# deezer/musicFPaugment

Measured on AMD Instinct MI355X. Metric: 8s/8kHz clips/sec (STFT+UNet+peak-pick), higher is better.
Workload: dtype bf16x3 (fp32 operands split into bf16 hi+lo, fp32 accumulate); 1 GPU; STFT(512/256,f64) -> UNet(1,1) eval forward (bf16x3 MFMA, formula weights) -> Audfprint peak-pick; 8 s / 8 kHz clips, 257x251 spectrograms; parallelism=clip-sharded x1, no data-path collective

## Files before the change

musicfpaugment_amd/csrc/mfpa_conv_tile.h:

```cpp
#pragma once
#include <hip/hip_runtime.h>

#include <type_traits>
#include <utility>

namespace mfpa_tile {

typedef float floatx16 __attribute__((ext_vector_type(16)));
typedef float floatx4 __attribute__((ext_vector_type(4)));
typedef float f32x4 __attribute__((ext_vector_type(4)));
typedef float f32x2 __attribute__((ext_vector_type(2)));
typedef __bf16 bf16x8 __attribute__((ext_vector_type(8)));
typedef __bf16 bf16x4 __attribute__((ext_vector_type(4)));
typedef __bf16 bf16x2 __attribute__((ext_vector_type(2)));

constexpr int KC = 32;

template <int CTRL>
__device__ __forceinline__ float dpp_row_add(float v) {
  return v + __int_as_float(__builtin_amdgcn_update_dpp(0, __float_as_int(v), CTRL, 0xf, 0xf, false));
}

template <int SLOTS, int LEFT, int I = 0>
__device__ __forceinline__ void pin_reads() {
  if constexpr (I < SLOTS && LEFT > 0) {
    constexpr int k = (LEFT + (SLOTS - I) - 1) / (SLOTS - I);
    __builtin_amdgcn_sched_group_barrier(0x008, 1, 0);
    __builtin_amdgcn_sched_group_barrier(0x100, k, 0);
    pin_reads<SLOTS, LEFT - k, I + 1>();
  }
}
constexpr int pin_read_slots(int slots, int left) {
  int used = 0;
  for (int i = 0; i < slots && left > 0; ++i) {
    left -= (left + (slots - i) - 1) / (slots - i);
    ++used;
  }
  return used;
}

__device__ __forceinline__ void split_bf16x3(f32x2 x, unsigned& hi, unsigned& lo) {
  hi = __builtin_bit_cast(unsigned, __builtin_convertvector(x, bf16x2));
  const f32x2 r = {x[0] - __uint_as_float(hi << 16), x[1] - __uint_as_float(hi & 0xffff0000u)};
  lo = __builtin_bit_cast(unsigned, __builtin_convertvector(r, bf16x2));
}

__device__ __forceinline__ void mfma_bf16x3(floatx16& acc, bf16x8 ah, bf16x8 al, bf16x8 bh, bf16x8 bl) {
  acc = __builtin_amdgcn_mfma_f32_32x32x16_bf16(al, bh, acc, 0, 0, 0);
  acc = __builtin_amdgcn_mfma_f32_32x32x16_bf16(ah, bl, acc, 0, 0, 0);
  acc = __builtin_amdgcn_mfma_f32_32x32x16_bf16(ah, bh, acc, 0, 0, 0);
}

template <int FIRST, class F, int... I, class... A>
__device__ __forceinline__ void each_index_impl(F&& f, std::integer_sequence<int, I...>, A&&... a) {
  (f(std::integral_constant<int, FIRST + I>{}, a...), ...);
}
template <int N, int FIRST = 0, class F, class... A>
__device__ __forceinline__ void each_index(F&& f, A&&... a) {
  each_index_impl<FIRST>(f, std::make_integer_sequence<int, N>{}, a...);
}

namespace role_split {
constexpr int PH = 8, PW = 32, HPW = PW + 2, HPH = PH + 2, HP = HPW * HPH;
constexpr int THREADS = 512, LTHREADS = 256;
constexpr int SPP = KC / 4;
constexpr int PPI = LTHREADS / SPP;
constexpr int A_F4 = (HP + PPI - 1) / PPI;
constexpr int HPS = A_F4 * PPI;
constexpr int PLANE = ((HPS * 16 + 255) / 256) * 256;
constexpr int HLS = 4 * PLANE + 256;
constexpr int STAGE = 2 * HLS;
constexpr int PT = 8;
constexpr int OUTBUF = PH * PW * 64 * 4;

__device__ __forceinline__ constexpr int plane_off(int hl, int kg) { return hl * HLS + kg * PLANE + (kg >> 1) * 128; }
}

}
```

musicfpaugment_amd/csrc/unet_up.hip:

```cpp
#include "mfpa_common.h"
#include "mfpa_conv_tile.h"
#include "mfpa_unet_args.h"

namespace mfpa_unet {
namespace {

using namespace mfpa_tile;
using namespace mfpa_tile::role_split;

constexpr int HALF = HPW / 2;
constexpr int LPH = PH / 2 + 2, LPW = PW / 2 + 2, LP = LPH * LPW;
constexpr int L_F4 = (LP + PPI - 1) / PPI;
constexpr int EPI_FLOATS = 64 + 16 * 64;

__device__ __forceinline__ int tile_of(int b, int i, int G, int ngrp) {
  if (ngrp == 1 && (G & 7) == 0) return i * G + (b & 7) * (G >> 3) + (b >> 3);
  return i * G + b;
}

__device__ __forceinline__ int bias_class(int v, int n2) { return v == 0 ? 0 : (v < n2 - 1 ? 1 : (v == n2 - 1 ? 2 : 3)); }

template <int PREC>
__global__ __launch_bounds__(THREADS, 1) void conv_up_kernel(UpArgs a) {
  extern __shared__ __attribute__((aligned(16))) char smem[];
// ... 129 lines not shown
        if (S.interior) each_index<A_F4>([&](auto IT) __attribute__((always_inline)) { issue_slot(S, ain, off0[decltype(IT)::value], std::true_type{}, SET, IT); });
        else each_index<A_F4>([&](auto IT) __attribute__((always_inline)) { issue_slot(S, ain, off0[decltype(IT)::value], std::false_type{}, SET, IT); });
      } else {
        if (S.interior) each_index<L_F4>([&](auto IT) __attribute__((always_inline)) { issue_slot(S, ain, off1[decltype(IT)::value], std::true_type{}, SET, IT); });
        else each_index<L_F4>([&](auto IT) __attribute__((always_inline)) { issue_slot(S, ain, off1[decltype(IT)::value], std::false_type{}, SET, IT); });
      }
    };
    auto split_all = [&](auto SET, int stage_off, bool from0) __attribute__((always_inline)) {
      each_index<L_F4>([&](auto IT) __attribute__((always_inline)) { split_slot(SET, IT, stage_off); });
      if (from0) each_index<A_F4 - L_F4, L_F4>([&](auto IT) __attribute__((always_inline)) { split_slot(SET, IT, stage_off); });
    };
    int qi = 0, qc = 0;
    Tile TQ = make_tile(tile_of(wgx, 0, G, ngrp));
    auto issue_next = [&](auto SET) __attribute__((always_inline)) {
      const Src S = make_src(TQ, qc);
      issue_all(S, TQ.ain, SET);
      if (++qc == nchunks) {
        qc = 0; ++qi;
        if (qi < owned) TQ = make_tile(tile_of(wgx, qi, G, ngrp));
      }
    };
    using SET0 = std::integral_constant<int, 0>;
    using SET1 = std::integral_constant<int, 1>;
    issue_next(SET0{});
    int par = 0;
    const int total = owned * nchunks;
    auto iteration = [&](int k, auto ISSUE_SET, auto SPLIT_SET) __attribute__((always_inline)) {
      if (k + 2 < total) issue_next(ISSUE_SET);
      __builtin_amdgcn_sched_barrier(0);
      if (k + 1 < total) split_all(SPLIT_SET, par * STAGE, ((k + 1) % nchunks) < nsk);
      if (k >= nchunks + 1 && (k - 1) % nchunks == 0) duty(tile_of(wgx, (k - 1) / nchunks - 1, G, ngrp));
      __syncthreads();
      par ^= 1;
    };
    for (int k = -1; k < total; k += 2) {
      iteration(k, SET1{}, SET0{});
      if (k + 1 < total) iteration(k + 1, SET0{}, SET1{});
    }
    __syncthreads();
    duty(tile_of(wgx, owned - 1, G, ngrp));
    return;
  }

  const int wm = wave & 1, wn = wave >> 1;
  const int p = lane & 15, g = lane >> 4;

  typedef typename std::conditional<PREC == 1, bf16x8, f32x4>::type frag_t;
  frag_t wq[4][2][2];
  const unsigned wrow = (unsigned)(a.Cout / 16), wcol = (unsigned)(n0 / 16 + 2 * wn);
  const __amdgpu_buffer_rsrc_t rs_skip = __builtin_amdgcn_make_buffer_rsrc(const_cast<float*>(a.w_skip), 0, (int)(9u * (unsigned)a.Cout * (unsigned)a.Cs * 4u), 0x00020000);
  const __amdgpu_buffer_rsrc_t rs_up = __builtin_amdgcn_make_buffer_rsrc(const_cast<float*>(a.w_up), 0, (int)(16u * (unsigned)a.Cout * (unsigned)a.Cl * 4u), 0x00020000);
  const int wlane = lane * 16;
  auto load_w_at = [&](__amdgpu_buffer_rsrc_t rs, unsigned blk, auto SLOT) __attribute__((always_inline)) {
    constexpr int slot = decltype(SLOT)::value;
    const int so = (int)__builtin_amdgcn_readfirstlane((int)(blk << 11));
    wq[slot][0][0] = __builtin_bit_cast(frag_t, __builtin_amdgcn_raw_buffer_load_b128(rs, wlane, so, 0));
    wq[slot][0][1] = __builtin_bit_cast(frag_t, __builtin_amdgcn_raw_buffer_load_b128(rs, wlane + 1024, so, 0));
    wq[slot][1][0] = __builtin_bit_cast(frag_t, __builtin_amdgcn_raw_buffer_load_b128(rs, wlane + 2048, so, 0));
    wq[slot][1][1] = __builtin_bit_cast(frag_t, __builtin_amdgcn_raw_buffer_load_b128(rs, wlane + 3072, so, 0));
  };
  auto load_w_skip = [&](int chunk, int tap, auto SLOT) __attribute__((always_inline)) {
    load_w_at(rs_skip, ((unsigned)tap * (unsigned)nsk + (unsigned)chunk) * wrow + wcol, SLOT);
  };
  auto load_w_up = [&](int chunk, int pair, int px, auto SLOT) __attribute__((always_inline)) {
    const unsigned t16 = (unsigned)((wm * 2 + px) * 4 + pair);
    load_w_at(rs_up, (t16 * (unsigned)nup + (unsigned)chunk) * wrow + wcol, SLOT);
  };
  struct XFrags { frag_t h[4], l[4]; };
  XFrags fx[2];
  const int pl0 = PREC == 1 ? plane_off(0, g) : plane_off(g >> 1, 2 * (g & 1));
  constexpr int SECOND = PREC == 1 ? HLS : PLANE;
  const int xb_skip = (wm * HPW + p) * 16 + pl0;
  const int xb_up = (wm * LPW + p) * 16 + pl0;
  constexpr int R_ALL = 0, R_FIRST = 1, R_SECOND = 2;
  auto read_at = [&](XFrags& f, const char* base, auto STRIDE, auto PART) __attribute__((always_inline)) {
    constexpr int stride = decltype(STRIDE)::value, part = decltype(PART)::value;
#pragma unroll
    for (int j = (part == R_SECOND ? 2 : 0); j < (part == R_FIRST ? 2 : 4); ++j) {
      const char* r = base + j * stride;
      f.l[j] = *reinterpret_cast<const frag_t*>(r + SECOND);
      f.h[j] = *reinterpret_cast<const frag_t*>(r);
    }
  };
  auto read_skip = [&](XFrags& f, const char* stage, auto TA, auto S, auto PART) __attribute__((always_inline)) {
    constexpr int ta = decltype(TA)::value, s = decltype(S)::value;
    read_at(f, stage + xb_skip + (ta * HPW + (s & 1) * HALF + (s >> 1)) * 16, std::integral_constant<int, 2 * HPW * 16>{}, PART);
  };
  auto read_up = [&](XFrags& f, const char* stage, auto TY, auto C, auto PART) __attribute__((always_inline)) {
    read_at(f, stage + xb_up + (decltype(TY)::value * LPW + decltype(C)::value) * 16, std::integral_constant<int, LPW * 16>{}, PART);
  };
  floatx4 acc[2][PT];
#pragma unroll
  for (int ct = 0; ct < 2; ++ct)
#pragma unroll
    for (int pt = 0; pt < PT; ++pt) acc[ct][pt] = floatx4{0.f, 0.f, 0.f, 0.f};
  floatx4 initv[2];
  auto mfma_half = [&](const XFrags& f, const frag_t (&w)[2][2], auto HALFI, auto FIRST) __attribute__((always_inline)) {
    constexpr int half = decltype(HALFI)::value;
    if constexpr (PREC == 0) {
#pragma unroll
      for (int s8 = 0; s8 < 8; ++s8)
#pragma unroll
        for (int ct = 0; ct < 2; ++ct)
#pragma unroll
          for (int i = 0; i < 4; ++i) {
            const float wv = (s8 < 4 ? w[ct][0] : w[ct][1])[s8 & 3], xv = (s8 < 4 ? f.h[i] : f.l[i])[s8 & 3];
            acc[ct][4 * half + i] = __builtin_amdgcn_mfma_f32_16x16x4f32(wv, xv, (decltype(FIRST)::value && s8 == 0) ? initv[ct] : acc[ct][4 * half + i], 0, 0, 0);
          }
      return;
    } else {
#pragma unroll
    for (int ct = 0; ct < 2; ++ct)
// ... 258 lines not shown
```

musicfpaugment_amd/csrc/unet_wd16.hip:

```cpp
#include "mfpa_common.h"
#include "mfpa_conv_tile.h"
#include "mfpa_unet_args.h"

namespace {

using namespace mfpa_tile;
using mfpa_unet::ConvArgs;

constexpr int wd16_bn(int wmw) { return 32 * (8 / wmw); }
constexpr bool wd16_persist(bool rows, int wmw, bool side, bool plain) { return wmw == 4 || (!rows && !side) || plain; }
template <int PH, int PW, bool IN16>
struct Wd16Lds {
  static constexpr int THREADS = 512;
  static constexpr int SPP = IN16 ? KC / 8 : KC / 4;
  static constexpr int HPW = PW + 2, HPH = PH + 2, HP = HPW * HPH;
  static constexpr int A_F4 = (HP * SPP + THREADS - 1) / THREADS;
  static constexpr int HPS = A_F4 * (THREADS / SPP);
  static constexpr int PLANE = ((HPS * 16 + 255) / 256) * 256;
  static constexpr int HLS = 4 * PLANE + 256;
  static constexpr int STAGE = 2 * HLS;
  static constexpr int TBL = 2 * A_F4 * THREADS;
  static constexpr int TBL_BYTES = 2 * ((HP * (KC / 4) + THREADS - 1) / THREADS) * THREADS * (int)sizeof(unsigned);
  static constexpr int RED = 2 * 256;
  static constexpr int epi_floats(int wmw) { return 2 * wd16_bn(wmw) + 64; }
  static constexpr int fixed_bytes(int wmw) { return 2 * STAGE + TBL_BYTES + epi_floats(wmw) * (int)sizeof(float); }
  __host__ __device__ static constexpr int plane_off(int hl, int kg) { return hl * HLS + kg * PLANE + (kg >> 1) * 128; }
  static_assert(TBL * (int)sizeof(unsigned) <= TBL_BYTES, "the kernel's table fits the launcher's");
};
static_assert(Wd16Lds<8, 32, false>::fixed_bytes(2) == 125184 && Wd16Lds<16, 16, false>::fixed_bytes(2) == 125184 &&
              Wd16Lds<8, 32, true>::fixed_bytes(2) == 125184 && Wd16Lds<16, 16, true>::fixed_bytes(2) == 125184, "LDS of the 128-channel tiles");
static_assert(Wd16Lds<8, 32, false>::fixed_bytes(4) == 124672 && Wd16Lds<8, 32, true>::fixed_bytes(4) == 124672, "LDS of the 64-channel tiles");


template <int PH, int PW, bool ROWS, int WMW = 2, bool SIDE = false, bool PLAIN = false, bool IN16 = false, bool AFF16 = false>
__global__ __launch_bounds__(512, 1) void conv_wd16_kernel(ConvArgs a) {
  static_assert(!IN16 || PLAIN, "a bf16 source feeds the plain-bf16 products");
  using G = Wd16Lds<PH, PW, IN16>;
  constexpr int SPP = G::SPP, HPW = G::HPW, HP = G::HP, A_F4 = G::A_F4, HLS = G::HLS, STAGE = G::STAGE, TBL = G::TBL;
  constexpr int ESZ = IN16 ? 2 : 4;
  constexpr int THREADS = G::THREADS, BN = wd16_bn(WMW), WPXW = 256 / WMW, TAPS = 9;
  static_assert((WMW == 2 || WMW == 4) && (!ROWS || WMW == 2), "wave grid");
  constexpr int BM = PH * PW;
  static_assert(BM == 256 && (PW == 32 || PW == 16), "two waves of 128 pixels: eight 16-pixel tiles each");
  constexpr int PT = WPXW / 16;
  static_assert(A_F4 <= TAPS - 3, "one halo staging slot per tap, taps 2 .. 7");

  extern __shared__ __attribute__((aligned(16))) char smem[];
  const int tid = threadIdx.x, lane = tid & 63, wave = tid >> 6;
  const int wm = wave % WMW, wn = __builtin_amdgcn_readfirstlane(wave / WMW);
  const int p = lane & 15, g = lane >> 4;

  constexpr bool PERSIST = wd16_persist(ROWS, WMW, SIDE, PLAIN);
  const int n0 = blockIdx.y * BN;
  const int Cin = a.C0 + a.C1;
  const int nchunks = Cin / KC;
  const int ntiles = a.tiles_x * a.tiles_y * a.B;

  const int aq = tid % SPP;
  unsigned* const aoffs0 = reinterpret_cast<unsigned*>(smem + 2 * STAGE);
#pragma unroll
  for (int it = 0; it < A_F4; ++it) {
    const int pix = tid / SPP + it * (THREADS / SPP);
    const int py = pix / HPW - 1, px = pix % HPW - 1;
    aoffs0[it * THREADS + tid] = (unsigned)((py * a.W + px) * a.C0 + (KC / SPP) * aq) * (unsigned)ESZ;
    aoffs0[(A_F4 + it) * THREADS + tid] = (unsigned)(((py - a.oy1) * a.W1 + (px - a.ox1)) * a.C1 + (KC / SPP) * aq) * (unsigned)ESZ;
  }
  const unsigned clip0 = (unsigned)a.H * (unsigned)a.W * (unsigned)a.C0 * (unsigned)ESZ, clip1 = (unsigned)a.H1 * (unsigned)a.W1 * (unsigned)a.C1 * (unsigned)ESZ;
  struct Tile { int b, y0, x0p; unsigned ain; unsigned t0, t1; };
  auto make_tile = [&](int t) __attribute__((always_inline)) {
    Tile T;
    int bx = __builtin_amdgcn_readfirstlane(t);
    const int tx = bx % a.tiles_x; bx /= a.tiles_x;
    const int ty = bx % a.tiles_y; bx /= a.tiles_y;
    T.b = bx; T.y0 = ty * PH; T.x0p = tx * PW; T.ain = 0;
    T.t0 = (unsigned)((T.y0 * a.W + T.x0p) * a.C0) * (unsigned)ESZ;
    T.t1 = (unsigned)((T.y0 * a.W1 + T.x0p) * a.C1) * (unsigned)ESZ;
#pragma unroll
    for (int it = 0; it < A_F4; ++it) {
      const int pix = tid / SPP + it * (THREADS / SPP);
      const int gy = T.y0 + pix / HPW - 1, gx = T.x0p + pix % HPW - 1;
      const bool in = pix < HP && gy >= 0 && gy < a.H && gx >= 0 && gx < a.W;
      const int y1 = gy - a.oy1, x1 = gx - a.ox1;
      const bool in1 = in && y1 >= 0 && y1 < a.H1 && x1 >= 0 && x1 < a.W1;
      T.ain |= (in ? 1u : 0u) << it | (in1 ? 1u : 0u) << (8 + it);
    }
    return T;
  };
  auto clip_rsrc = [&](const float* base, int b, unsigned clip_bytes) __attribute__((always_inline)) {
    const char* pb = reinterpret_cast<const char*>(base) + (size_t)b * clip_bytes;
    return __builtin_amdgcn_make_buffer_rsrc(const_cast<char*>(pb), 0, base != nullptr ? (int)clip_bytes : 0, 0x00020000);
  };
  int tile = blockIdx.x;
  Tile S = make_tile(tile);
  int eb = S.b, ey0 = S.y0, ex0p = S.x0p;
  float* aff = reinterpret_cast<float*>(smem + 2 * STAGE + TBL * sizeof(unsigned));
  if (a.in_scale0 != nullptr) {
    for (int i = tid; i < a.C0; i += THREADS) {
      aff[i] = a.in_scale0[i];
      aff[a.C0 + i] = a.in_shift0[i];
    }
    __syncthreads();
  }
  float* const epi = aff + (a.in_scale0 ? 2 * a.C0 : 0) + (a.w1x1 ? G::RED : 0);
  for (int i = tid; i < BN; i += THREADS) {
    epi[i] = a.scale ? a.scale[n0 + i] : 1.f;
    epi[BN + i] = a.shift ? a.shift[n0 + i] : 0.f;
  }
  if (a.w1x1 != nullptr && tid < 64) epi[2 * BN + tid] = a.w1x1[tid];
  constexpr int AHALF = (A_F4 + 1) / 2, AREGS = ROWS ? AHALF : A_F4;
  f32x4 areg[AREGS];
  auto load_a_range = [&](int chunk, auto FIRST, auto COUNT) __attribute__((always_inline)) {
    constexpr int first = decltype(FIRST)::value, count = decltype(COUNT)::value;
    const int c0 = chunk * KC;
    const bool from0 = c0 < a.C0;
    const auto rs = clip_rsrc(from0 ? a.x0 : a.x1, S.b, from0 ? clip0 : clip1);
    const unsigned toff = from0 ? S.t0 + (unsigned)c0 * (unsigned)ESZ : S.t1 + (unsigned)(c0 - a.C0) * (unsigned)ESZ;
    const unsigned* ao = aoffs0 + (from0 ? 0 : A_F4 * THREADS) + tid;
#pragma unroll
    for (int it = first; it < first + count && it < A_F4; ++it)
      areg[it % AREGS] = __builtin_bit_cast(f32x4, __builtin_amdgcn_raw_buffer_load_b128(rs, (int)(ao[it * THREADS] + toff), 0, 0));
  };
  auto load_a = [&](int chunk) __attribute__((always_inline)) {
    load_a_range(chunk, std::integral_constant<int, 0>{}, std::integral_constant<int, AREGS>{});
  };
  auto preload_offsets = [&](int chunk) __attribute__((always_inline)) {
    const unsigned* ao = aoffs0 + (chunk * KC < a.C0 ? 0 : A_F4 * THREADS) + tid;
#pragma unroll
    for (int it = 0; it < A_F4; ++it) areg[it % AREGS][0] = __uint_as_float(ao[it * THREADS]);
  };
  auto load_a_pre = [&](int chunk) __attribute__((always_inline)) {
    const int c0 = chunk * KC;
    const bool from0 = c0 < a.C0;
// ... 9 lines not shown
    const int c0 = chunk * KC;
    const bool inside = (S.ain >> ((c0 < a.C0 ? 0 : 8) + it)) & 1u;
    f32x4 v = areg[it % AREGS];
    if (!inside) v = f32x4{0.f, 0.f, 0.f, 0.f};
    if constexpr (IN16) {
      if (AFF16 && a.in_scale0 != nullptr && c0 < a.C0 && inside) {
        float f[8];
#pragma unroll
        for (int k = 0; k < 4; ++k) {
          const unsigned u = __float_as_uint(v[k]);
          f[2 * k] = __uint_as_float(u << 16);
          f[2 * k + 1] = __uint_as_float(u & 0xffff0000u);
        }
        const float* scp = aff + c0 + 8 * aq;
        const float* shp = aff + a.C0 + c0 + 8 * aq;
        const f32x4 sc0 = *reinterpret_cast<const f32x4*>(scp), sc1 = *reinterpret_cast<const f32x4*>(scp + 4);
        const f32x4 sh0 = *reinterpret_cast<const f32x4*>(shp), sh1 = *reinterpret_cast<const f32x4*>(shp + 4);
#pragma unroll
        for (int k = 0; k < 8; ++k) {
          const float y = f[k] * (k < 4 ? sc0[k & 3] : sc1[k & 3]) + (k < 4 ? sh0[k & 3] : sh1[k & 3]);
          f[k] = y > 0.f ? y : 0.f;
        }
        if (a.drop_thresh) {
          const int gy = S.y0 + pix / HPW - 1, gx = S.x0p + pix % HPW - 1;
          const unsigned long long e0 = (((unsigned long long)S.b * a.H + gy) * a.W + gx) * a.C0 + c0 + 8 * aq;
#pragma unroll
          for (int k = 0; k < 8; ++k) f[k] = mfpa_keep(a.drop_seed, a.drop_thresh, e0 + k) ? f[k] * a.drop_scale : 0.f;
        }
#pragma unroll
        for (int k = 0; k < 4; ++k) {
          bf16x2 h2;
          h2[0] = (__bf16)f[2 * k];
          h2[1] = (__bf16)f[2 * k + 1];
          v[k] = __builtin_bit_cast(float, h2);
        }
      }
      *reinterpret_cast<f32x4*>(stage + G::plane_off(0, aq) + pix * 16) = v;
      if constexpr (SIDE && AFF16) {
        const int py = pix / HPW, px = pix % HPW;
        if (a.x0_bf16 != nullptr && c0 < a.C0 && inside && py >= 1 && py <= PH && px >= 1 && px <= PW && blockIdx.y == 0) {
          const size_t e = (size_t)S.b * a.H * a.W * a.C0 + ((aoffs0[it * THREADS + tid] + S.t0) >> 1) + c0;
          *reinterpret_cast<f32x4*>(a.x0_bf16 + e) = v;
        }
      }
      return;
    }
    if (a.in_scale0 != nullptr && c0 < a.C0 && inside) {
      const f32x4 sc = *reinterpret_cast<const f32x4*>(aff + c0 + 4 * aq);
      const f32x4 sh = *reinterpret_cast<const f32x4*>(aff + a.C0 + c0 + 4 * aq);
      v = v * sc + sh;
#pragma unroll
      for (int k = 0; k < 4; ++k) v[k] = v[k] > 0.f ? v[k] : 0.f;
      if (a.drop_thresh) {
        const int gy = S.y0 + pix / HPW - 1, gx = S.x0p + pix % HPW - 1;
        const unsigned long long e0 = (((unsigned long long)S.b * a.H + gy) * a.W + gx) * a.C0 + c0 + 4 * aq;
#pragma unroll
        for (int k = 0; k < 4; ++k) v[k] = mfpa_keep(a.drop_seed, a.drop_thresh, e0 + k) ? v[k] * a.drop_scale : 0.f;
      }
    }
    bf16x4 hi, lo;
#pragma unroll
    for (int k = 0; k < 4; ++k) {
      hi[k] = (__bf16)v[k];
      lo[k] = (__bf16)(v[k] - (float)hi[k]);
    }
    char* at = stage + G::plane_off(0, aq >> 1) + pix * 16 + 8 * (aq & 1);
    *reinterpret_cast<bf16x4*>(at) = hi;
    if constexpr (!PLAIN) *reinterpret_cast<bf16x4*>(at + HLS) = lo;
    if constexpr (SIDE) {
      const int py = pix / HPW, px = pix % HPW;
      const bool interior = inside && py >= 1 && py <= PH && px >= 1 && px <= PW && blockIdx.y == 0;
      if (a.x0_bf16 != nullptr && c0 < a.C0 && interior) {
        const size_t e = (size_t)S.b * a.H * a.W * a.C0 + ((aoffs0[it * THREADS + tid] + S.t0) >> 2) + c0;
        *reinterpret_cast<bf16x4*>(a.x0_bf16 + e) = hi;
      }
      if (a.x1_bf16 != nullptr && c0 >= a.C0 && interior) {
        const size_t e = (size_t)S.b * a.H1 * a.W1 * a.C1 + ((aoffs0[(A_F4 + it) * THREADS + tid] + S.t1) >> 2) + (c0 - a.C0);
        *reinterpret_cast<bf16x4*>(a.x1_bf16 + e) = hi;
      }
    }
  };

  bf16x8 wq[3][2][2];
  auto w_frag = [&](int tap, int chunk) __attribute__((always_inline)) {
    return reinterpret_cast<const char*>(a.w) +
           ((((size_t)tap * nchunks + chunk) * (size_t)(a.Cout / 16) + (size_t)(n0 / 16 + 2 * wn)) << 11) + lane * 16;
  };
  auto load_w = [&](int chunk, int tap, auto SLOT) __attribute__((always_inline)) {
    constexpr int slot = decltype(SLOT)::value;
    const char* wb = w_frag(tap, chunk);
    wq[slot][0][0] = *reinterpret_cast<const bf16x8*>(wb);
    if constexpr (!PLAIN) wq[slot][0][1] = *reinterpret_cast<const bf16x8*>(wb + 1024);
    wq[slot][1][0] = *reinterpret_cast<const bf16x8*>(wb + 2048);
    if constexpr (!PLAIN) wq[slot][1][1] = *reinterpret_cast<const bf16x8*>(wb + 3072);
  };

  struct XFrags { bf16x8 h[4], l[4]; };
  XFrags fx0, fx1;
  const int xbase = (((wm * WPXW + p) / PW) * HPW + ((wm * WPXW + p) % PW)) * 16 + G::plane_off(0, g);
  auto tile_disp = [](int pt) { return (PW == 32) ? ((pt >> 1) * HPW + (pt & 1) * 16) * 16 : pt * HPW * 16; };
  auto read_x = [&](XFrags& f, const char* stage, int tap_off, int half) __attribute__((always_inline)) {
#pragma unroll
    for (int i = 0; i < 4; ++i) {
      const char* r = stage + xbase + tile_disp(4 * half + i) + tap_off;
      if constexpr (!PLAIN) f.l[i] = *reinterpret_cast<const bf16x8*>(r + HLS);
      f.h[i] = *reinterpret_cast<const bf16x8*>(r);
    }
  };
  floatx4 acc[2][PT];
#pragma unroll
  for (int ct = 0; ct < 2; ++ct)
#pragma unroll
    for (int pt = 0; pt < PT; ++pt) acc[ct][pt] = floatx4{0.f, 0.f, 0.f, 0.f};
  auto mfma_half = [&](const XFrags& f, const bf16x8 (&w)[2][2], int half) __attribute__((always_inline)) {
    if constexpr (!PLAIN) {
#pragma unroll
    for (int ct = 0; ct < 2; ++ct)
#pragma unroll
      for (int i = 0; i < 4; ++i) acc[ct][4 * half + i] = __builtin_amdgcn_mfma_f32_16x16x32_bf16(w[ct][1], f.h[i], acc[ct][4 * half + i], 0, 0, 0);
#pragma unroll
    for (int ct = 0; ct < 2; ++ct)
#pragma unroll
      for (int i = 0; i < 4; ++i) acc[ct][4 * half + i] = __builtin_amdgcn_mfma_f32_16x16x32_bf16(w[ct][0], f.l[i], acc[ct][4 * half + i], 0, 0, 0);
    }
#pragma unroll
    for (int ct = 0; ct < 2; ++ct)
#pragma unroll
      for (int i = 0; i < 4; ++i) acc[ct][4 * half + i] = __builtin_amdgcn_mfma_f32_16x16x32_bf16(w[ct][0], f.h[i], acc[ct][4 * half + i], 0, 0, 0);
  };
  using S0 = std::integral_constant<int, 0>;
  using S1 = std::integral_constant<int, 1>;
  constexpr int N_R = PLAIN ? 4 : 8, N_M = PLAIN ? 8 : 24;
  constexpr int N_W = PLAIN ? 2 : 4;
  auto tap_body = [&](auto TAP, int chunk) __attribute__((always_inline)) {
    constexpr int tap = decltype(TAP)::value;
    constexpr int ntap = (tap + 1) % TAPS;
    constexpr int tap_off = ((tap / 3) * HPW + (tap % 3)) * 16, ntap_off = ((ntap / 3) * HPW + (ntap % 3)) * 16;
    const int chunk_n = chunk + 1 < nchunks ? chunk + 1 : (PERSIST ? 0 : chunk);
    const char* cur = smem + (chunk & 1) * STAGE;
    const char* nxt = (tap == TAPS - 1) ? smem + ((chunk + 1) & 1) * STAGE : cur;
    read_x(fx1, cur, tap_off, 1);
    mfma_half(fx0, wq[tap % 3], 0);
    load_w((tap + 2 >= TAPS) ? chunk_n : chunk, (tap + 2) % TAPS, std::integral_constant<int, (tap + 2) % 3>{});
    pin_reads<N_M - 1, N_R>();
    constexpr int used_a = pin_read_slots(N_M - 1, N_R);
    __builtin_amdgcn_sched_group_barrier(0x008, 1, 0);
    __builtin_amdgcn_sched_group_barrier(0x020, N_W, 0);
// ... 39 lines not shown
    const char* nxt = (tap == TAPS - 1) ? smem + ((chunk + 1) & 1) * STAGE : cur;
    if (tap == TAPS - 1) {
      __syncthreads();
      __builtin_amdgcn_sched_barrier(0);
    }
    if (tap == 0) load_a_pre(chunk_n);
    if (tap == TAPS - 1) preload_offsets(chunk + 2 < nchunks ? chunk + 2 : chunk + 1 < nchunks ? 0 : 1 < nchunks ? 1 : 0);
    read_x(par ? fx0 : fx1, nxt, ntap_off, 0);
    mfma_half(par ? fx1 : fx0, wq[tap % 3], 0);
    load_w((tap + 2 >= TAPS) ? chunk_n : chunk, (tap + 2) % TAPS, std::integral_constant<int, (tap + 2) % 3>{});
    if constexpr (tap >= 2 && tap - 2 < A_F4) {
      split_slot(std::integral_constant<int, tap - 2>{}, chunk_n, smem + ((chunk + 1) & 1) * STAGE);
#pragma unroll
      for (int i = 0; i < N_R; ++i) {
        __builtin_amdgcn_sched_group_barrier(0x008, 1, 0);
        __builtin_amdgcn_sched_group_barrier(0x100, 1, 0);
        __builtin_amdgcn_sched_group_barrier(0x002, 2, 0);
      }
#pragma unroll
      for (int i = 0; i < N_W; ++i) {
        if constexpr (!PLAIN) __builtin_amdgcn_sched_group_barrier(0x008, 1, 0);
        __builtin_amdgcn_sched_group_barrier(0x020, 1, 0);
        __builtin_amdgcn_sched_group_barrier(0x002, 2, 0);
      }
#pragma unroll
      for (int i = 0; i < 2; ++i) {
        __builtin_amdgcn_sched_group_barrier(0x008, 2, 0);
        __builtin_amdgcn_sched_group_barrier(0x002, 4, 0);
        __builtin_amdgcn_sched_group_barrier(0x200, 1, 0);
      }
      if constexpr (N_M - N_R - 8 > 0) __builtin_amdgcn_sched_group_barrier(0x008, N_M - N_R - 8, 0);
    } else {
#pragma unroll
      for (int i = 0; i < N_R; ++i) {
        __builtin_amdgcn_sched_group_barrier(0x008, 1, 0);
        __builtin_amdgcn_sched_group_barrier(0x100, 1, 0);
      }
#pragma unroll
      for (int i = 0; i < N_W; ++i) {
        __builtin_amdgcn_sched_group_barrier(0x008, 1, 0);
        __builtin_amdgcn_sched_group_barrier(0x020, 1, 0);
      }
      if constexpr (N_M - N_R - N_W > 0) __builtin_amdgcn_sched_group_barrier(0x008, N_M - N_R - N_W, 0);
    }
    __builtin_amdgcn_sched_barrier(0);
  };

  constexpr int R = BM / 2 / PW, HV = PW / 16;
  bf16x8 wr[2][3][2][2];
  constexpr int NU = (R + 2) * HV, NB = (PW == 32) ? 4 : 5;
  static_assert(NU % NB == 0, "static ring indices");
  auto load_wr1 = [&](int chunk, auto DX, auto PAR, auto DY) __attribute__((always_inline)) {
    constexpr int dx = decltype(DX)::value, par = decltype(PAR)::value, dy = decltype(DY)::value;
    const char* wb = w_frag(dy * 3 + dx, chunk);
    wr[par][dy][0][0] = *reinterpret_cast<const bf16x8*>(wb);
    if constexpr (!PLAIN) wr[par][dy][0][1] = *reinterpret_cast<const bf16x8*>(wb + 1024);
    wr[par][dy][1][0] = *reinterpret_cast<const bf16x8*>(wb + 2048);
    if constexpr (!PLAIN) wr[par][dy][1][1] = *reinterpret_cast<const bf16x8*>(wb + 3072);
  };
  struct XUnit { bf16x8 h, l; };
  XUnit xu[NB];
  auto read_unit = [&](XUnit& f, const char* stage, int u, int dx) __attribute__((always_inline)) {
    const char* r = stage + xbase + ((u / HV) * HPW + (u % HV) * 16 + dx) * 16;
    if constexpr (!PLAIN) f.l = *reinterpret_cast<const bf16x8*>(r + HLS);
    f.h = *reinterpret_cast<const bf16x8*>(r);
  };
  auto mfma_unit = [&](auto U, const XUnit& f, auto PAR) __attribute__((always_inline)) {
    constexpr int h = decltype(U)::value / HV, hv = decltype(U)::value % HV, par = decltype(PAR)::value;
#pragma unroll
    for (int term = PLAIN ? 2 : 0; term < 3; ++term)
#pragma unroll
      for (int dy = 0; dy < 3; ++dy) {
        if (h - dy < 0 || h - dy >= R) continue;
#pragma unroll
        for (int ct = 0; ct < 2; ++ct) {
          floatx4& c = acc[ct][(h - dy) * HV + hv];
          c = __builtin_amdgcn_mfma_f32_16x16x32_bf16(wr[par][dy][ct][term == 0 ? 1 : 0], term == 1 ? f.l : f.h, c, 0, 0, 0);
        }
      }
  };
  auto unit_mfmas = [](int u) { const int h = u / HV; int n = 0; for (int dy = 0; dy < 3; ++dy) n += (h - dy >= 0 && h - dy < R) ? 1 : 0; return n * (PLAIN ? 2 : 6); };
  constexpr int BARU = NU - NB + 1;
  constexpr int SA = NU / 2, SB = BARU - AHALF;
  static_assert(SA + AHALF < NU && SB >= 0, "staging schedule");
  auto unit_step = [&](auto U, auto DX, auto PAR, int chunk) __attribute__((always_inline)) {
    constexpr int u = decltype(U)::value, dx = decltype(DX)::value, par = decltype(PAR)::value;
    constexpr int n_m = unit_mfmas(u);
    const int chunk_n = chunk + 1 < nchunks ? chunk + 1 : (PERSIST ? 0 : chunk);
    const char* cur = smem + (chunk & 1) * STAGE;
    char* nxs = smem + ((chunk + 1) & 1) * STAGE;
    if constexpr (u == BARU && dx == 2) {
      __syncthreads();
      __builtin_amdgcn_sched_barrier(0);
    }
    constexpr int pu = u + NB - 1;
    if constexpr (pu < NU) read_unit(xu[pu % NB], cur, pu, dx);
    else read_unit(xu[pu % NB], dx == 2 ? nxs : cur, pu - NU, (dx + 1) % 3);
    mfma_unit(U, xu[u % NB], PAR);
    constexpr int split_it = dx == 1 ? u - SA : dx == 2 ? AHALF + u - SB : -1;
    constexpr bool do_split = (dx == 1 && u >= SA && u < SA + AHALF) || (dx == 2 && u >= SB && u < SB + AHALF && split_it < A_F4);
    if constexpr (u == 0 && dx == 0) load_a_range(chunk_n, std::integral_constant<int, 0>{}, std::integral_constant<int, AHALF>{});
    if constexpr (u == SA + AHALF && dx == 1) load_a_range(chunk_n, std::integral_constant<int, AHALF>{}, std::integral_constant<int, AHALF>{});
    if constexpr (u >= 1 && u <= 3) {
      if constexpr (dx < 2) load_wr1(chunk, std::integral_constant<int, (dx + 1) % 3>{}, std::integral_constant<int, par ^ 1>{}, std::integral_constant<int, u - 1>{});
      else load_wr1(chunk_n, std::integral_constant<int, 0>{}, std::integral_constant<int, par ^ 1>{}, std::integral_constant<int, u - 1>{});
    }
    if constexpr (do_split) split_slot(std::integral_constant<int, split_it>{}, chunk_n, nxs);
// ... 3 lines not shown
#pragma unroll
      for (int i = 1; i < n_m; ++i) {
        __builtin_amdgcn_sched_group_barrier(0x002, (24 + n_m - 2) / (n_m - 1), 0);
        __builtin_amdgcn_sched_group_barrier(0x008, 1, 0);
      }
      __builtin_amdgcn_sched_group_barrier(0x200, 1, 0);
    } else if constexpr (PLAIN && u >= 1 && u <= 3) {
      __builtin_amdgcn_sched_group_barrier(0x020, 2, 0);
      if constexpr (n_m - 1 > 0) __builtin_amdgcn_sched_group_barrier(0x008, n_m - 1, 0);
    } else if constexpr (do_split) {
      __builtin_amdgcn_sched_group_barrier(0x002, 6, 0);
#pragma unroll
      for (int i = 0; i < 4; ++i) {
        __builtin_amdgcn_sched_group_barrier(0x008, 1, 0);
        __builtin_amdgcn_sched_group_barrier(0x002, 6, 0);
      }
      __builtin_amdgcn_sched_group_barrier(0x200, 2, 0);
      if constexpr (n_m - 5 > 0) __builtin_amdgcn_sched_group_barrier(0x008, n_m - 5, 0);
    } else if constexpr (u >= 1 && u <= 3) {
#pragma unroll
      for (int i = 0; i < 4; ++i) {
        __builtin_amdgcn_sched_group_barrier(0x008, 1, 0);
        __builtin_amdgcn_sched_group_barrier(0x020, 1, 0);
      }
      if constexpr (n_m - 5 > 0) __builtin_amdgcn_sched_group_barrier(0x008, n_m - 5, 0);
    } else {
      if constexpr (n_m - 1 > 0) __builtin_amdgcn_sched_group_barrier(0x008, n_m - 1, 0);
    }
    __builtin_amdgcn_sched_barrier(0);
  };
  auto period = [&](auto DX, auto PAR, int chunk) __attribute__((always_inline)) {
    each_index<NU>(unit_step, DX, PAR, chunk);
  };

  if constexpr (ROWS) {
    f32x4 keep[AREGS];
    load_a_range(0, std::integral_constant<int, AHALF>{}, std::integral_constant<int, AHALF>{});
#pragma unroll
    for (int i = 0; i < AREGS; ++i) keep[i] = areg[i];
    load_a_range(0, std::integral_constant<int, 0>{}, std::integral_constant<int, AHALF>{});
    each_index<3>([&](auto DY) __attribute__((always_inline)) { load_wr1(0, S0{}, S0{}, DY); });
    each_index<AHALF>(split_slot, 0, smem);
#pragma unroll
    for (int i = 0; i < AREGS; ++i) areg[i] = keep[i];
    each_index<A_F4 - AHALF, AHALF>(split_slot, 0, smem);
    static_assert(A_F4 <= 2 * AHALF, "two halves of staging slots");
  } else {
    load_a(0);
    load_w(0, 0, S0{});
    load_w(0, 1, S1{});
    each_index<A_F4>(split_slot, 0, smem);
    preload_offsets(1 < nchunks ? 1 : 0);
  }
  auto epilogue = [&]() __attribute__((always_inline)) {
  #pragma unroll
    for (int ct = 0; ct < 2; ++ct) {
      const int chl = wn * 32 + ct * 16 + 4 * g;
      const f32x4 sc = *reinterpret_cast<const f32x4*>(epi + chl);
      const f32x4 sh = *reinterpret_cast<const f32x4*>(epi + BN + chl);
  #pragma unroll
      for (int pt = 0; pt < PT; ++pt)
  #pragma unroll
        for (int j = 0; j < 4; ++j) {
          float v = acc[ct][pt][j] * sc[j] + sh[j];
          if (a.relu) v = v > 0.f ? v : 0.f;
          acc[ct][pt][j] = v;
        }
    }
    if (SIDE && a.stats_part != nullptr) {
      float vm[PT];
  #pragma unroll
      for (int pt = 0; pt < PT; ++pt) {
        const int m = wm * WPXW + pt * 16 + p;
        vm[pt] = (ey0 + m / PW < a.yH && ex0p + m % PW < a.yW) ? 1.f : 0.f;
      }
      float* row = a.stats_part + ((size_t)tile * WMW + wm) * 2 * a.Cout + n0 + wn * 32 + 4 * g;
  #pragma unroll
      for (int ct = 0; ct < 2; ++ct) {
        f32x4 sv = {0.f, 0.f, 0.f, 0.f}, qv = {0.f, 0.f, 0.f, 0.f};
        if (!AFF16 && a.bz != nullptr) {
          const int ch = n0 + wn * 32 + ct * 16 + 4 * g;
          const f32x4 bsc = *reinterpret_cast<const f32x4*>(a.bz_scale + ch), bsh = *reinterpret_cast<const f32x4*>(a.bz_shift + ch);
          const f32x4 bmu = *reinterpret_cast<const f32x4*>(a.bz_mean + ch), bis = *reinterpret_cast<const f32x4*>(a.bz_invstd + ch);
          f32x4 zzs[PT];
          auto zoff = [&](int pt) __attribute__((always_inline)) {
            const int m = wm * WPXW + pt * 16 + p;
            const int gy = min(ey0 + m / PW, a.yH - 1), gx = min(ex0p + m % PW, a.yW - 1);
            return (((size_t)eb * a.yH + gy) * a.yW + gx) * (size_t)a.Cout + ch;
          };
          if (a.bz16) {
            f32x2 raw[PT];
  #pragma unroll
            for (int pt = 0; pt < PT; ++pt) raw[pt] = *reinterpret_cast<const f32x2*>(reinterpret_cast<const __bf16*>(a.bz) + zoff(pt));
  #pragma unroll
            for (int pt = 0; pt < PT; ++pt) {
              const unsigned u0 = __float_as_uint(raw[pt][0]), u1 = __float_as_uint(raw[pt][1]);
              zzs[pt] = f32x4{__uint_as_float(u0 << 16), __uint_as_float(u0 & 0xffff0000u), __uint_as_float(u1 << 16), __uint_as_float(u1 & 0xffff0000u)};
            }
          } else {
  #pragma unroll
            for (int pt = 0; pt < PT; ++pt) zzs[pt] = *reinterpret_cast<const f32x4*>(a.bz + zoff(pt));
          }
  #pragma unroll
          for (int pt = 0; pt < PT; ++pt) {
            const f32x4 zz = zzs[pt];
  #pragma unroll
            for (int j = 0; j < 4; ++j) {
              const float gg = (zz[j] * bsc[j] + bsh[j] > 0.f) ? acc[ct][pt][j] * vm[pt] : 0.f;
              sv[j] += gg;
              qv[j] += gg * ((zz[j] - bmu[j]) * bis[j]);
            }
          }
        } else {
  #pragma unroll
        for (int pt = 0; pt < PT; ++pt)
  #pragma unroll
          for (int j = 0; j < 4; ++j) {
            const float v = acc[ct][pt][j] * vm[pt];
            sv[j] += v;
            qv[j] += v * v;
          }
        }
  #pragma unroll
        for (int j = 0; j < 4; ++j) {
          sv[j] = dpp_row_add<0x118>(dpp_row_add<0x114>(dpp_row_add<0x112>(dpp_row_add<0x111>(sv[j]))));
          qv[j] = dpp_row_add<0x118>(dpp_row_add<0x114>(dpp_row_add<0x112>(dpp_row_add<0x111>(qv[j]))));
        }
        if (p == 15) {
          *reinterpret_cast<f32x4*>(row + ct * 16) = sv;
          *reinterpret_cast<f32x4*>(row + a.Cout + ct * 16) = qv;
        }
      }
    }
    if (a.y != nullptr || (SIDE && IN16 && a.y_bf16 != nullptr)) {
      char* yb = reinterpret_cast<char*>(a.y + (size_t)eb * a.yH * a.yW * a.Cout);
  #pragma unroll
      for (int pt = 0; pt < PT; ++pt) {
        const int m = wm * WPXW + pt * 16 + p;
        const int gy = ey0 + m / PW, gx = ex0p + m % PW;
        if (gy < a.yH && gx < a.yW) {
          char* yp = yb + (((unsigned)gy * (unsigned)a.yW + (unsigned)gx) * (unsigned)a.Cout + (unsigned)(n0 + wn * 32 + 4 * g)) * 4u;
          if (a.y != nullptr) {
  #pragma unroll
          for (int ct = 0; ct < 2; ++ct) {
            f32x4 o;
  #pragma unroll
            for (int j = 0; j < 4; ++j) o[j] = acc[ct][pt][j];
            *reinterpret_cast<f32x4*>(yp + ct * 64) = o;
          }
          }
          if (SIDE && a.y_bf16 != nullptr) {
            __bf16* hp = a.y_bf16 + (((size_t)eb * a.yH + gy) * a.yW + gx) * (size_t)a.Cout + n0 + wn * 32 + 4 * g;
  #pragma unroll
            for (int ct = 0; ct < 2; ++ct) {
              bf16x4 h;
  #pragma unroll
              for (int j = 0; j < 4; ++j) h[j] = (__bf16)acc[ct][pt][j];
              *reinterpret_cast<bf16x4*>(hp + ct * 16) = h;
            }
          }
        }
      }
    }
    if (a.y_pool != nullptr) {
      const int Ho = a.H / 2, Wo = a.W / 2;
      constexpr int ROWSTEP = (PW == 32) ? 2 : 1;
  #pragma unroll
      for (int ct = 0; ct < 2; ++ct)
  #pragma unroll
        for (int pt = 0; pt < PT; ++pt) {
          const int row = pt / ROWSTEP;
          if (row & 1) continue;
          f32x4 v;
  #pragma unroll
          for (int j = 0; j < 4; ++j) {
            const float t = fmaxf(acc[ct][pt][j], acc[ct][pt + ROWSTEP][j]);
            const float o = __int_as_float(__builtin_amdgcn_update_dpp(0, __float_as_int(t), 0xB1, 0xf, 0xf, true));
            v[j] = fmaxf(t, o);
          }
          const int m = wm * WPXW + pt * 16 + p;
          const int py = (ey0 + m / PW) / 2, px = (ex0p + m % PW) / 2;
          if (!(p & 1) && py < Ho && px < Wo)
            *reinterpret_cast<f32x4*>(a.y_pool + (((size_t)eb * Ho + py) * Wo + px) * a.Cout + n0 + wn * 32 + ct * 16 + 4 * g) = v;
        }
    }
  
    if constexpr (WMW == 4) {
      if (a.w1x1 != nullptr) {
        float* red = reinterpret_cast<float*>(smem + 2 * STAGE + TBL * sizeof(unsigned)) + (a.in_scale0 ? 2 * a.C0 : 0);
        const f32x4 w0 = *reinterpret_cast<const f32x4*>(epi + 2 * BN + wn * 32 + 4 * g);
        const f32x4 w1 = *reinterpret_cast<const f32x4*>(epi + 2 * BN + wn * 32 + 16 + 4 * g);
  #pragma unroll
        for (int pt = 0; pt < PT; ++pt) {
          float v = 0.f;
  #pragma unroll
          for (int j = 0; j < 4; ++j) v += acc[0][pt][j] * w0[j] + acc[1][pt][j] * w1[j];
          v += __shfl_xor(v, 16);
          v += __shfl_xor(v, 32);
          if (g == 0) red[wn * 256 + wm * WPXW + pt * 16 + p] = v;
        }
        __syncthreads();
        if (tid < 256) {
          const int gy = ey0 + tid / PW, gx = ex0p + tid % PW;
          if (gy < a.H && gx < a.W) a.y1x1[((size_t)eb * a.H + gy) * a.W + gx] = red[tid] + red[256 + tid] + a.b1x1;
        }
        __syncthreads();
      }
    }
  };

  __syncthreads();
  if constexpr (ROWS) {
#pragma unroll
    for (int u = 0; u < NB - 1; ++u) read_unit(xu[u], smem, u, 0);
  } else {
    read_x(fx0, smem, 0, 0);
  }
  for (;;) {
    const int tile_n = tile + (int)gridDim.x;
    const bool has_next = PERSIST && tile_n < ntiles;
    const Tile N = PERSIST ? make_tile(has_next ? tile_n : tile) : S;
    if constexpr (ROWS) {
      using D0 = std::integral_constant<int, 0>;
      using D1 = std::integral_constant<int, 1>;
      using D2 = std::integral_constant<int, 2>;
      for (int chunk = 0; chunk < nchunks; chunk += 2) {
        period(D0{}, S0{}, chunk);
        period(D1{}, S1{}, chunk);
        period(D2{}, S0{}, chunk);
        if (PERSIST && chunk + 2 >= nchunks) S = N;
        period(D0{}, S1{}, chunk + 1);
        period(D1{}, S0{}, chunk + 1);
        period(D2{}, S1{}, chunk + 1);
      }
    } else if constexpr (WMW == 4) {
      for (int chunk = 0; chunk < nchunks; chunk += 2) {
        each_index<TAPS>(tap_body4, S0{}, chunk);
        if (chunk + 2 >= nchunks) S = N;
        each_index<TAPS>(tap_body4, S1{}, chunk + 1);
      }
    } else {
      for (int chunk = 0; chunk < nchunks; ++chunk) {
        if (PERSIST && chunk + 1 >= nchunks) S = N;
        each_index<TAPS>(tap_body, chunk);
      }
    }
    epilogue();
    if (!has_next) break;
    tile = tile_n; eb = S.b; ey0 = S.y0; ex0p = S.x0p;
#pragma unroll
    for (int ct = 0; ct < 2; ++ct)
#pragma unroll
      for (int pt = 0; pt < PT; ++pt) acc[ct][pt] = floatx4{0.f, 0.f, 0.f, 0.f};
  }
}

}

namespace mfpa_unet {

const int CONV_WD16_ROWS = 512;
void conv_wd16_tile(int W, int Cout, mfpa_conv_route* t) {
  t->wmw = Cout % 128 ? 4 : 2; t->bn = 32 * (8 / t->wmw);
  t->pw = (t->wmw == 2 && W <= 16) ? 16 : 32; t->ph = 256 / t->pw;
}

template <int PH, int PW, bool ROWS, int WMW, bool SIDE, bool PLAIN, bool IN16, bool AFF16>
int launch_wd16(ConvArgs& a, hipStream_t s) {
  using G = Wd16Lds<PH, PW, IN16>;
  const size_t lds = (size_t)G::fixed_bytes(WMW) +
                     (a.in_scale0 ? (size_t)2 * a.C0 * sizeof(float) : 0) +
                     (a.w1x1 ? G::RED * sizeof(float) : 0);
  dim3 grid((unsigned)((long long)a.tiles_x * a.tiles_y * a.B), (unsigned)(a.Cout / wd16_bn(WMW)));
  if constexpr (wd16_persist(ROWS, WMW, SIDE, PLAIN)) {
    const int cus = mfpa_current_device_cus();
    const unsigned per = (unsigned)((cus > 0 ? cus : 256) / (int)grid.y);
    if (per >= 1 && grid.x > per && ((a.C0 + a.C1) / KC) % 2 == 0) grid.x = per;
  }
  hipLaunchKernelGGL((conv_wd16_kernel<PH, PW, ROWS, WMW, SIDE, PLAIN, IN16, AFF16>), grid, dim3(G::THREADS), lds, s, a);
  MFPA_CHECK_LAUNCH();
  return MFPA_OK;
}
#define MFPA_WD16_INSTANTIATE(...) template int launch_wd16<__VA_ARGS__>(ConvArgs&, hipStream_t);
MFPA_WD16_FORMS(MFPA_WD16_INSTANTIATE)

}
```

Measured before the change: 5256 clips/s.

## Make row-pipelined wd16 conv persistent with register-lean rematerialization and buffer weight loads

Enables the persistent tile loop for the ROWS variant of the wd16 conv kernel when it has no side output. For that path, lane/tid-derived indices, epilogue scalars and zero constants are passed through empty asm barriers so the compiler rematerializes them rather than keeping them live across the main loop, which is meant to cut register pressure. The next tile descriptor is now computed at the point of use instead of being held across the loop. Weight fragment loads move from flat global pointers to raw buffer loads with a scalar offset via a shared helper, also used in the up kernel. This trades a few recomputed instructions for fewer live registers and less per-tile launch overhead, with the risk of spilling or worse scheduling if the gamble fails.

```diff
diff --git a/musicfpaugment_amd/csrc/mfpa_conv_tile.h b/musicfpaugment_amd/csrc/mfpa_conv_tile.h
--- a/musicfpaugment_amd/csrc/mfpa_conv_tile.h
+++ b/musicfpaugment_amd/csrc/mfpa_conv_tile.h
@@ -60,6 +60,23 @@
   each_index_impl<FIRST>(f, std::make_integer_sequence<int, N>{}, a...);
 }
 
+__device__ __forceinline__ __amdgpu_buffer_rsrc_t wfrag_rsrc(const void* base, unsigned long long bytes) {
+  return __builtin_amdgcn_make_buffer_rsrc(const_cast<void*>(base), 0, bytes >> 32 ? -1 : (int)(unsigned)bytes, 0x00020000);
+}
+template <bool LO = true, class T>
+__device__ __forceinline__ void load_wfrags(T (&w)[2][2], __amdgpu_buffer_rsrc_t rs, int wlane, unsigned blk) {
+  const int so = (int)__builtin_amdgcn_readfirstlane((int)(blk << 11));
+  w[0][0] = __builtin_bit_cast(T, __builtin_amdgcn_raw_buffer_load_b128(rs, wlane, so, 0));
+  if constexpr (LO) w[0][1] = __builtin_bit_cast(T, __builtin_amdgcn_raw_buffer_load_b128(rs, wlane + 1024, so, 0));
+  w[1][0] = __builtin_bit_cast(T, __builtin_amdgcn_raw_buffer_load_b128(rs, wlane + 2048, so, 0));
+  if constexpr (LO) w[1][1] = __builtin_bit_cast(T, __builtin_amdgcn_raw_buffer_load_b128(rs, wlane + 3072, so, 0));
+}
+template <bool LO = true, class T>
+__device__ __forceinline__ void load_wfrags_any(T (&w)[2][2], const void* image, unsigned long long bytes, int wlane, unsigned blk) {
+  const unsigned long long skip = (unsigned long long)(blk >> 20) << 31;
+  load_wfrags<LO>(w, wfrag_rsrc(reinterpret_cast<const char*>(image) + skip, bytes - skip), wlane, blk & 0xfffffu);
+}
+
 namespace role_split {
 constexpr int PH = 8, PW = 32, HPW = PW + 2, HPH = PH + 2, HP = HPW * HPH;
 constexpr int THREADS = 512, LTHREADS = 256;
diff --git a/musicfpaugment_amd/csrc/unet_up.hip b/musicfpaugment_amd/csrc/unet_up.hip
--- a/musicfpaugment_amd/csrc/unet_up.hip
+++ b/musicfpaugment_amd/csrc/unet_up.hip
@@ -205,12 +205,7 @@
   const __amdgpu_buffer_rsrc_t rs_up = __builtin_amdgcn_make_buffer_rsrc(const_cast<float*>(a.w_up), 0, (int)(16u * (unsigned)a.Cout * (unsigned)a.Cl * 4u), 0x00020000);
   const int wlane = lane * 16;
   auto load_w_at = [&](__amdgpu_buffer_rsrc_t rs, unsigned blk, auto SLOT) __attribute__((always_inline)) {
-    constexpr int slot = decltype(SLOT)::value;
-    const int so = (int)__builtin_amdgcn_readfirstlane((int)(blk << 11));
-    wq[slot][0][0] = __builtin_bit_cast(frag_t, __builtin_amdgcn_raw_buffer_load_b128(rs, wlane, so, 0));
-    wq[slot][0][1] = __builtin_bit_cast(frag_t, __builtin_amdgcn_raw_buffer_load_b128(rs, wlane + 1024, so, 0));
-    wq[slot][1][0] = __builtin_bit_cast(frag_t, __builtin_amdgcn_raw_buffer_load_b128(rs, wlane + 2048, so, 0));
-    wq[slot][1][1] = __builtin_bit_cast(frag_t, __builtin_amdgcn_raw_buffer_load_b128(rs, wlane + 3072, so, 0));
+    load_wfrags(wq[decltype(SLOT)::value], rs, wlane, blk);
   };
   auto load_w_skip = [&](int chunk, int tap, auto SLOT) __attribute__((always_inline)) {
     load_w_at(rs_skip, ((unsigned)tap * (unsigned)nsk + (unsigned)chunk) * wrow + wcol, SLOT);
diff --git a/musicfpaugment_amd/csrc/unet_wd16.hip b/musicfpaugment_amd/csrc/unet_wd16.hip
--- a/musicfpaugment_amd/csrc/unet_wd16.hip
+++ b/musicfpaugment_amd/csrc/unet_wd16.hip
@@ -8,7 +8,7 @@
 using mfpa_unet::ConvArgs;
 
 constexpr int wd16_bn(int wmw) { return 32 * (8 / wmw); }
-constexpr bool wd16_persist(bool rows, int wmw, bool side, bool plain) { return wmw == 4 || (!rows && !side) || plain; }
+constexpr bool wd16_persist(bool rows, int wmw, bool side, bool plain) { return wmw == 4 || !side || plain; }
 template <int PH, int PW, bool IN16>
 struct Wd16Lds {
   static constexpr int THREADS = 512;
@@ -51,6 +51,15 @@
   const int p = lane & 15, g = lane >> 4;
 
   constexpr bool PERSIST = wd16_persist(ROWS, WMW, SIDE, PLAIN);
+  constexpr bool LEAN = PERSIST && ROWS && !PLAIN;
+  auto fresh = [](int v) __attribute__((always_inline)) {
+    if constexpr (LEAN) asm volatile("" : "+v"(v));
+    return v;
+  };
+  auto fresh_s = [](int v) __attribute__((always_inline)) {
+    if constexpr (LEAN) asm volatile("" : "+s"(v));
+    return v;
+  };
   const int n0 = blockIdx.y * BN;
   const int Cin = a.C0 + a.C1;
   const int nchunks = Cin / KC;
@@ -75,9 +84,10 @@
     T.b = bx; T.y0 = ty * PH; T.x0p = tx * PW; T.ain = 0;
     T.t0 = (unsigned)((T.y0 * a.W + T.x0p) * a.C0) * (unsigned)ESZ;
     T.t1 = (unsigned)((T.y0 * a.W1 + T.x0p) * a.C1) * (unsigned)ESZ;
+    const int pix0 = fresh(tid) / SPP;
 #pragma unroll
     for (int it = 0; it < A_F4; ++it) {
-      const int pix = tid / SPP + it * (THREADS / SPP);
+      const int pix = pix0 + it * (THREADS / SPP);
       const int gy = T.y0 + pix / HPW - 1, gx = T.x0p + pix % HPW - 1;
       const bool in = pix < HP && gy >= 0 && gy < a.H && gx >= 0 && gx < a.W;
       const int y1 = gy - a.oy1, x1 = gx - a.ox1;
@@ -193,7 +203,8 @@
 #pragma unroll
       for (int k = 0; k < 4; ++k) v[k] = v[k] > 0.f ? v[k] : 0.f;
       if (a.drop_thresh) {
-        const int gy = S.y0 + pix / HPW - 1, gx = S.x0p + pix % HPW - 1;
+        const int dpix = fresh(tid) / SPP + it * (THREADS / SPP);
+        const int gy = S.y0 + dpix / HPW - 1, gx = S.x0p + dpix % HPW - 1;
         const unsigned long long e0 = (((unsigned long long)S.b * a.H + gy) * a.W + gx) * a.C0 + c0 + 4 * aq;
 #pragma unroll
         for (int k = 0; k < 4; ++k) v[k] = mfpa_keep(a.drop_seed, a.drop_thresh, e0 + k) ? v[k] * a.drop_scale : 0.f;
@@ -223,17 +234,12 @@
   };
 
   bf16x8 wq[3][2][2];
-  auto w_frag = [&](int tap, int chunk) __attribute__((always_inline)) {
-    return reinterpret_cast<const char*>(a.w) +
-           ((((size_t)tap * nchunks + chunk) * (size_t)(a.Cout / 16) + (size_t)(n0 / 16 + 2 * wn)) << 11) + lane * 16;
-  };
+  const unsigned wrow = (unsigned)(a.Cout / 16), wcol = (unsigned)(n0 / 16 + 2 * wn);
+  const unsigned long long wbytes = ((unsigned long long)TAPS * (unsigned)nchunks * wrow) << 11;
+  const int wlane = lane * 16;
+  auto w_blk = [&](int tap, int chunk) __attribute__((always_inline)) { return ((unsigned)tap * (unsigned)nchunks + (unsigned)chunk) * wrow + wcol; };
   auto load_w = [&](int chunk, int tap, auto SLOT) __attribute__((always_inline)) {
-    constexpr int slot = decltype(SLOT)::value;
-    const char* wb = w_frag(tap, chunk);
-    wq[slot][0][0] = *reinterpret_cast<const bf16x8*>(wb);
-    if constexpr (!PLAIN) wq[slot][0][1] = *reinterpret_cast<const bf16x8*>(wb + 1024);
-    wq[slot][1][0] = *reinterpret_cast<const bf16x8*>(wb + 2048);
-    if constexpr (!PLAIN) wq[slot][1][1] = *reinterpret_cast<const bf16x8*>(wb + 3072);
+    load_wfrags_any<!PLAIN>(wq[decltype(SLOT)::value], a.w, wbytes, wlane, w_blk(tap, chunk));
   };
 
   struct XFrags { bf16x8 h[4], l[4]; };
@@ -379,7 +385,7 @@
   static_assert(NU % NB == 0, "static ring indices");
   auto load_wr1 = [&](int chunk, auto DX, auto PAR, auto DY) __attribute__((always_inline)) {
     constexpr int dx = decltype(DX)::value, par = decltype(PAR)::value, dy = decltype(DY)::value;
-    const char* wb = w_frag(dy * 3 + dx, chunk);
+    const char* wb = reinterpret_cast<const char*>(a.w) + ((size_t)w_blk(dy * 3 + dx, chunk) << 11) + wlane;
     wr[par][dy][0][0] = *reinterpret_cast<const bf16x8*>(wb);
     if constexpr (!PLAIN) wr[par][dy][0][1] = *reinterpret_cast<const bf16x8*>(wb + 1024);
     wr[par][dy][1][0] = *reinterpret_cast<const bf16x8*>(wb + 2048);
@@ -489,7 +495,7 @@
     each_index<A_F4>(split_slot, 0, smem);
     preload_offsets(1 < nchunks ? 1 : 0);
   }
-  auto epilogue = [&]() __attribute__((always_inline)) {
+  auto epilogue = [&](const int p, const int g, const int wm) __attribute__((always_inline)) {
   #pragma unroll
     for (int ct = 0; ct < 2; ++ct) {
       const int chl = wn * 32 + ct * 16 + 4 * g;
@@ -571,12 +577,13 @@
     }
     if (a.y != nullptr || (SIDE && IN16 && a.y_bf16 != nullptr)) {
       char* yb = reinterpret_cast<char*>(a.y + (size_t)eb * a.yH * a.yW * a.Cout);
+      const unsigned eyW = (unsigned)fresh_s(a.yW), eCout = (unsigned)fresh_s(a.Cout);
   #pragma unroll
       for (int pt = 0; pt < PT; ++pt) {
         const int m = wm * WPXW + pt * 16 + p;
         const int gy = ey0 + m / PW, gx = ex0p + m % PW;
         if (gy < a.yH && gx < a.yW) {
-          char* yp = yb + (((unsigned)gy * (unsigned)a.yW + (unsigned)gx) * (unsigned)a.Cout + (unsigned)(n0 + wn * 32 + 4 * g)) * 4u;
+          char* yp = yb + (((unsigned)gy * eyW + (unsigned)gx) * eCout + (unsigned)(n0 + wn * 32 + 4 * g)) * 4u;
           if (a.y != nullptr) {
   #pragma unroll
           for (int ct = 0; ct < 2; ++ct) {
@@ -656,7 +663,7 @@
   for (;;) {
     const int tile_n = tile + (int)gridDim.x;
     const bool has_next = PERSIST && tile_n < ntiles;
-    const Tile N = PERSIST ? make_tile(has_next ? tile_n : tile) : S;
+    const Tile N = PERSIST && !LEAN ? make_tile(has_next ? tile_n : tile) : S;
     if constexpr (ROWS) {
       using D0 = std::integral_constant<int, 0>;
       using D1 = std::integral_constant<int, 1>;
@@ -665,7 +672,7 @@
         period(D0{}, S0{}, chunk);
         period(D1{}, S1{}, chunk);
         period(D2{}, S0{}, chunk);
-        if (PERSIST && chunk + 2 >= nchunks) S = N;
+        if (PERSIST && chunk + 2 >= nchunks) S = LEAN ? make_tile(has_next ? tile_n : tile) : N;
         period(D0{}, S1{}, chunk + 1);
         period(D1{}, S0{}, chunk + 1);
         period(D2{}, S1{}, chunk + 1);
@@ -682,13 +689,15 @@
         each_index<TAPS>(tap_body, chunk);
       }
     }
-    epilogue();
+    epilogue(fresh(lane) & 15, fresh(lane) >> 4, (fresh(tid) >> 6) % WMW);
     if (!has_next) break;
     tile = tile_n; eb = S.b; ey0 = S.y0; ex0p = S.x0p;
+    float zero = 0.f;
+    if constexpr (LEAN) asm volatile("" : "+v"(zero));
 #pragma unroll
     for (int ct = 0; ct < 2; ++ct)
 #pragma unroll
-      for (int pt = 0; pt < PT; ++pt) acc[ct][pt] = floatx4{0.f, 0.f, 0.f, 0.f};
+      for (int pt = 0; pt < PT; ++pt) acc[ct][pt] = floatx4{zero, zero, zero, zero};
   }
 }
 
```

Result: no change. 5279 clips/s (median of 6 runs) (+0.4%).
